# yanzq95/DHD

Measured on AMD Instinct MI355X. Metric: samples/sec (6-cam fwd+bwd) DHD-S view-transform hot path, higher is better.
Workload: dtype f32

## Files before the change

dhd_amd/csrc/sfa_stage.hip:

```cpp
#include <stdlib.h>

#include <type_traits>

#include "sfa_gemm_cu.h"
#include "sfa_gemm_pair.h"
#include "sfa_half.h"
#include "sfa_mfma.h"

using namespace dhd_sfa;

namespace {

constexpr int kEwBlock = 256;
constexpr int kPlaneChunks = 4;
constexpr int kPwBlock = 256;
constexpr int kPwStep = 16;
constexpr int kWgBlock = 512;
constexpr int kWgStride = 33;
constexpr int kWgWorkers = 256;
__host__ __device__ inline long long wg_first_step(long long n, long long w, long long W) { return n * w / W; }
__host__ __device__ inline int wg_owner(long long n, long long s, long long W) { return (int)(((s + 1) * W + n - 1) / n) - 1; }
struct WgFirstStep {
  __host__ __device__ long long operator()(long long n, long long w, long long W) const { return wg_first_step(n, w, W); }
};
inline int wgrad_blocks(int c) { const int ot = c == 128 ? 128 : 256; return (c / ot) * (c / ot); }
inline int wgrad_workers(int c) { const int nob = wgrad_blocks(c); return kWgWorkers / nob > 0 ? kWgWorkers / nob : 1; }
constexpr int kBwdFoldDefault = 7;

__device__ __forceinline__ float block_sum(float v, float* sm) {
  v = group_sum(v, DHD_WAVE);
  const int lane = threadIdx.x & 63, wv = threadIdx.x >> 6;
  __syncthreads();
  if (lane == 0) sm[wv] = v;
  __syncthreads();
  float t = 0.f;
  for (int k = 0; k < (int)(blockDim.x / DHD_WAVE); ++k) t += sm[k];
  return t;
}

template <class TS> constexpr bool kHalfStorage = !std::is_same_v<TS, float>;
template <class TS> constexpr bool kStreamAll = kHalfStorage<TS>;
template <class TS> constexpr int kWideInFlight = kHalfStorage<TS> ? 2 : 1;
template <class TS> constexpr bool kFoldPairwise = !kHalfStorage<TS>;

template <int N> __device__ __forceinline__ void chunk_range(int hw, int* lo, int* hi) {
  static_assert(N == 4 || N == 8, "16 bytes of float32 or of a half type");
  const int n = hw >> (N == 8 ? 3 : 2), per = (n + kPlaneChunks - 1) / kPlaneChunks;
  *lo = blockIdx.x * per;
  *hi = min(n, *lo + per);
}

template <class TO, int N> struct IoVec {
  static constexpr bool k16 = N == kVec16<TO>;
  static_assert(k16 || (N == 4 && sizeof(TO) == 2), "16 bytes, or four elements of a half type");
  using raw = std::conditional_t<k16, raw16<TO>, u32x2>;
  static __device__ __forceinline__ raw ld(const TO* base, size_t i) { return __builtin_nontemporal_load(reinterpret_cast<const raw*>(base) + i); }
  static __device__ __forceinline__ void widen(raw w, float* v) {
    if constexpr (k16) {
      widen16<TO>(w, v);
    } else {
      const f32x2 a = Pair<TO>::widen(w.x), b = Pair<TO>::widen(w.y);
      v[0] = a.x; v[1] = a.y; v[2] = b.x; v[3] = b.y;
    }
  }
  static __device__ __forceinline__ void store(TO* base, size_t i, const float* v) {
    if constexpr (k16) {
      Vec16<TO, true>::store(base, i, v);
    } else {
      typedef TO t4 __attribute__((ext_vector_type(4)));
      const t4 h = {(TO)v[0], (TO)v[1], (TO)v[2], (TO)v[3]};
      __builtin_nontemporal_store(h, reinterpret_cast<t4*>(base) + i);
    }
  }
};

template <int N> __device__ __forceinline__ float tree_sum(const float* v) {
  if constexpr (N == 4) return (v[0] + v[1]) + (v[2] + v[3]);
  else return tree_sum<N / 2>(v) + tree_sum<N / 2>(v + N / 2);
}

template <class TS> __device__ __forceinline__ float fold_sum(float acc, const float* a) {
  if constexpr (kFoldPairwise<TS>) return acc + tree_sum<kVec16<TS>>(a);
#pragma unroll
  for (int j = 0; j < kVec16<TS>; ++j) acc += a[j];
  return acc;
}
template <class TS, class D> __device__ __forceinline__ float fold_dot(float acc, const float* a, D d) {
  if constexpr (kFoldPairwise<TS>) {
    static_assert(kVec16<TS> == 4, "the pairwise fold is written for four elements");
    return acc + ((a[0] * d(0) + a[1] * d(1)) + (a[2] * d(2) + a[3] * d(3)));
  }
#pragma unroll
  for (int j = 0; j < kVec16<TS>; ++j) acc = fmaf(a[j], d(j), acc);
  return acc;
}

template <int K, class Load, class Body> __device__ __forceinline__ void for_each_vector(int lo, int hi, Load load, Body body) {
  int i = lo + threadIdx.x;
  if constexpr (K == 2) {
    for (; i + kEwBlock < hi; i += 2 * kEwBlock) {
      const auto u = load(i), w = load(i + kEwBlock);
      body(u, i);
      body(w, i + kEwBlock);
    }
    if (i < hi) body(load(i), i);
  } else {
    for (; i < hi; i += kEwBlock) body(load(i), i);
  }
}


template <class TS>
__device__ __forceinline__ void plane_mean_block(const TS* __restrict__ x, float* __restrict__ part, int hw, float* sm) {
  constexpr int N = kVec16<TS>;
  using X = Vec16<TS, true>;
  const size_t plane = blockIdx.y;
  const TS* p = x + plane * hw;
  int lo, hi;
  chunk_range<N>(hw, &lo, &hi);
  float a0 = 0.f, a1 = 0.f;
  int i = lo + threadIdx.x;
  for (; i + kEwBlock < hi; i += 2 * kEwBlock) {
    float v[N], w[N];
    X::load(p, i, v);
    X::load(p, (size_t)i + kEwBlock, w);
    a0 += tree_sum<N>(v);
    a1 += tree_sum<N>(w);
  }
  if (i < hi) {
    float v[N];
    X::load(p, i, v);
    a0 += tree_sum<N>(v);
  }
  const float tot = block_sum(a0 + a1, sm);
  if (threadIdx.x == 0) part[plane * kPlaneChunks + blockIdx.x] = tot;
}

__global__ __launch_bounds__(kEwBlock) void plane_mean_kernel(const float* __restrict__ x, float* __restrict__ part, int hw) {
  __shared__ float sm[kEwBlock / DHD_WAVE];
  plane_mean_block(x, part, hw, sm);
}

constexpr int kFcBlock = 1024;
__global__ __launch_bounds__(kFcBlock) void fc_forward_kernel(const float* __restrict__ part, const float* __restrict__ w1,
                                                              const float* __restrict__ b1, const float* __restrict__ w2,
                                                              const float* __restrict__ b2, float* __restrict__ s,
                                                              float* __restrict__ hbuf, float* __restrict__ a,
                                                              float* __restrict__ tab, int c, int r, int hw,
                                                              int* __restrict__ ticks, int n_ticks) {
  extern __shared__ float sh[];
  if (blockIdx.x == 0)
    for (int i = threadIdx.x; i < n_ticks; i += kFcBlock) ticks[i] = 0;
  float* ss = sh;
  float* hh = sh + 2 * c;
  const int b = blockIdx.x, c2 = 2 * c;
  for (int i = threadIdx.x; i < c2; i += kFcBlock) {
    const float* q = part + ((size_t)b * c2 + i) * kPlaneChunks;
    float v = ((q[0] + q[1]) + (q[2] + q[3])) / (float)hw;
    ss[i] = v;
    s[(size_t)b * c2 + i] = v;
  }
  __syncthreads();
  const int lane = threadIdx.x & 63, wv = threadIdx.x >> 6;
  for (int j0 = wv * 4; j0 < r; j0 += 4 * (kFcBlock / DHD_WAVE)) {
    float acc[4] = {0.f, 0.f, 0.f, 0.f};
    for (int i = lane; i < c2; i += DHD_WAVE) {
      const float sv = ss[i];
#pragma unroll
      for (int q = 0; q < 4; ++q)
        if (j0 + q < r) acc[q] = fmaf(w1[(size_t)(j0 + q) * c2 + i], sv, acc[q]);
    }
#pragma unroll
    for (int q = 0; q < 4; ++q) {
      const float t = group_sum(acc[q], DHD_WAVE);
      if (lane == 0 && j0 + q < r) {
        const float v = fmaxf(t + b1[j0 + q], 0.f);
        hh[j0 + q] = v;
        hbuf[(size_t)b * r + j0 + q] = v;
      }
    }
// ... 1337 lines not shown
      constexpr int OT = decltype(ot_c)::value;
      if constexpr (!std::is_same<TS, float>::value) {
        const size_t shmem = (size_t)2 * 4 * 2 * (OT / 32) * 64 * 16;
        return launch_lds<pw_wgrad_h_kernel<TS, OT, V::two, V::relu>>(grid, block, shmem, shmem, st, a0, a1, acoef, a_bs, b0, b1, bcoef,
                                                                     b_bs, partial, c, hw, b, workers);
      } else if (p.wgrad == Wgrad::w3) {
        const size_t shmem = (size_t)2 * 2 * 2 * (OT / 32) * 2 * 64 * 16;
        if (fold.mode != 0) {
          if (nob != 1 || fold.mode != (V::two ? 2 : 1)) return (int)DHD_EUNSUPPORTED;
          return launch_lds<pw_wgrad3_kernel<OT, false, V::two, V::relu, V::two ? 2 : 1>>(grid, block, shmem, shmem, st, a0, a1, acoef, a_bs, b0, b1,
                                                                                         bcoef, b_bs, partial, c, hw, b, workers, fold.aux,
                                                                                         fold.mean, fold.rows);
        }
        return launch_lds<pw_wgrad3_kernel<OT, true, V::two, V::relu>>(grid, block, shmem, shmem, st, a0, a1, acoef, a_bs, b0, b1, bcoef,
                                                                      b_bs, partial, c, hw, b, workers, static_cast<const float*>(nullptr),
                                                                      static_cast<const float*>(nullptr), static_cast<float*>(nullptr));
      } else if (p.wgrad == Wgrad::w6) {
        const size_t shmem = (size_t)2 * 2 * (OT / 32) * 3 * 64 * 16;
        return launch_lds<pw_wgrad6_kernel<OT, true, V::two, V::relu>>(grid, block, shmem, shmem, st, a0, a1, acoef, a_bs, b0, b1, bcoef,
                                                                      b_bs, partial, c, hw, b, workers);
      } else {
        const size_t shmem = (size_t)4 * OT * kWgStride * sizeof(float);
        return launch_lds<pw_wgrad_kernel<OT, true, V::two, V::relu>>(grid, block, shmem, shmem, st, a0, a1, acoef, a_bs, b0, b1, bcoef,
                                                                     b_bs, partial, c, hw, b, workers);
      }
    };
    return ot == 128 ? run(IntC<128>{}) : run(IntC<256>{});
  });
  if (rc != DHD_OK) return rc;
  const int n = c * c;
  hipLaunchKernelGGL(wgrad_reduce_kernel, dim3(dhd_cdiv(n, DHD_WAVE)), dim3(kEwBlock), 0, st, partial, gw, n, workers);
  DHD_LAUNCH_CHECK();
  return DHD_OK;
}

template <class TS>
int launch_mean_pack(const Plan& p, const TS* x, const float* w1, const float* w2, void* const dst[4], float* mean_part, int b,
                     int c, int hw, hipStream_t st) {
  const int blocks_each = dhd_cdiv((c / 32) * (c / 16) * 64, kEwBlock);
  if (p.pack == Pack::cu || p.pack == Pack::res || p.pack == Pack::cuh) {
    PackJob job;
    job.w[0] = w1; job.w[1] = w2;
    for (int i = 0; i < 4; ++i) job.dst[i] = static_cast<u32x4*>(dst[i]);
    job.c = c; job.nt = p.nt; job.cob = p.cob; job.cu = p.pack == Pack::cu ? 1 : 0;
    job.blocks_each = blocks_each;
    const dim3 grid(kPlaneChunks, b * 2 * c + dhd_cdiv(4 * blocks_each, kPlaneChunks));
    hipLaunchKernelGGL(plane_mean_pack_kernel<TS>, grid, dim3(kEwBlock), 0, st, x, mean_part, hw, b * 2 * c, job);
    DHD_LAUNCH_CHECK();
    return DHD_OK;
  }
  if constexpr (std::is_same_v<TS, float>) {
    hipLaunchKernelGGL(plane_mean_kernel, dim3(kPlaneChunks, b * 2 * c), dim3(kEwBlock), 0, st, x, mean_part, hw);
    DHD_LAUNCH_CHECK();
    for (int i = 0; i < 4; ++i) {
      const float* wi = i & 1 ? w2 : w1;
      if (p.pack == Pack::six)
        hipLaunchKernelGGL(pack_weight6_kernel, dim3(blocks_each), dim3(kEwBlock), 0, st, wi, i >> 1, static_cast<u32x4*>(dst[i]), c, p.cot);
      else
        hipLaunchKernelGGL(pack_weight_kernel, dim3(dhd_cdiv(c * c, kEwBlock)), dim3(kEwBlock), 0, st, wi, i >> 1, static_cast<float*>(dst[i]),
                           c, p.cot);
      DHD_LAUNCH_CHECK();
    }
    return DHD_OK;
  }
  return DHD_EINVAL;
}

template <class TS, class TO>
int stage_forward(const Plan& p, const TS* x, const dhd_sfa_weights* w, TO* out, void* saved, void* scratch, int b, int c, int hw,
                  int lo, int hi, double* sync, hipStream_t st) {
  const int r = w->hidden;
  const SavedLayout S = saved_layout(b, c, hw, r, p.storage);
  const ScratchLayout T = scratch_layout(b, c, hw, r, p.storage);
  char* sv = static_cast<char*>(saved);
  char* sc = static_cast<char*>(scratch);
  auto SF = [&](size_t off) { return reinterpret_cast<float*>(sv + off); };
  auto TF = [&](size_t off) { return reinterpret_cast<float*>(sc + off); };
  TS* y1 = reinterpret_cast<TS*>(sv + S.y1);
  TS* y2 = reinterpret_cast<TS*>(sv + S.y2);
  float* stat_part = p.fused_stats ? TF(T.stat_part) : nullptr;
  const dim3 planes(kPlaneChunks, b * c), per_ch(dhd_cdiv(c, kEwBlock));
  const size_t cs = (size_t)c * hw;
  int stat_rows = 0, rc;
  struct Bn {
    const float *shift, *gamma, *beta;
    float *run_mean, *run_var;
    float momentum, eps;
    long long* batches;
    float *mean, *rstd, *scsh;
    double* loc;
  };
  const Bn bn1 = {w->conv1_b, w->bn1_w, w->bn1_b, w->bn1_mean, w->bn1_var, w->momentum1, w->eps1,
                  reinterpret_cast<long long*>(w->bn1_batches), SF(S.mean1), SF(S.rstd1), SF(S.scsh1), reinterpret_cast<double*>(sv + S.loc1)};
  const Bn bn2 = {w->conv2_b, w->bn2_w, w->bn2_b, w->bn2_mean, w->bn2_var, w->momentum2, w->eps2,
                  reinterpret_cast<long long*>(w->bn2_batches), SF(S.mean2), SF(S.rstd2), SF(S.scsh2), reinterpret_cast<double*>(sv + S.loc2)};
  auto publish = [&](const Bn& n, float* tab) {
    hipLaunchKernelGGL(bn_stats_finalize_kernel, dim3(c / 4), dim3(kEwBlock), 0, st, TF(T.stat_part), stat_rows, n.shift, n.gamma, n.beta,
                       n.run_mean, n.run_var, n.momentum, n.eps, n.mean, n.rstd, n.scsh, tab, b, c, hw, sync, n.loc, nullptr, nullptr);
  };
  auto coef = [&](const Bn& n, const TS* y, float* tab) {
    if (!w->training) {
      hipLaunchKernelGGL(bn_eval_coef_kernel, per_ch, dim3(kEwBlock), 0, st, n.gamma, n.beta, n.run_mean, n.run_var, n.eps, n.mean, n.rstd,
                         n.scsh, tab, b, c);
    } else if (p.fused_stats) {
      hipLaunchKernelGGL(bn_stats_finalize_kernel, dim3(c / 4), dim3(kEwBlock), 0, st, TF(T.stat_part), stat_rows, n.shift, n.gamma, n.beta,
                         n.run_mean, n.run_var, n.momentum, n.eps, n.mean, n.rstd, n.scsh, tab, b, c, hw, nullptr, nullptr, sync, n.batches);
    } else if constexpr (std::is_same<TS, float>::value) {
      hipLaunchKernelGGL(moments_kernel, planes, dim3(kEwBlock), 0, st, y, TF(T.part), c, hw);
      hipLaunchKernelGGL(bn_train_finalize_kernel, per_ch, dim3(kEwBlock), 0, st, TF(T.part), b * kPlaneChunks, y, hw, n.gamma, n.beta,
                         n.run_mean, n.run_var, n.momentum, n.eps, n.mean, n.rstd, n.scsh, tab, b, c, hw, n.batches);
    }
  };
  if (sync && !p.fused_stats) return DHD_EUNSUPPORTED;

  if (lo <= 0) {
    void* const dst[4] = {sc + T.wp1, sc + T.wp2, sv + S.wp1t, sv + S.wp2t};
    rc = launch_mean_pack(p, x, w->conv1_w, w->conv2_w, dst, TF(T.mean_part), b, c, hw, st);
    if (rc != DHD_OK) return rc;
    hipLaunchKernelGGL(fc_forward_kernel, dim3(b), dim3(kFcBlock), (size_t)(2 * c + r) * sizeof(float), st, TF(T.mean_part), w->fc1_w,
                       w->fc1_b, w->fc2_w, w->fc2_b, SF(S.s), SF(S.h), SF(S.a1), SF(S.tab_a), c, r, hw, reinterpret_cast<int*>(sv + S.tick),
                       2 * c + kTickWords);
    DHD_LAUNCH_CHECK();
    rc = launch_gemm(p, GemmCall<TS>{kConv1, x, x + cs, 2 * cs, c, SF(S.tab_a), sc + T.wp1, w->conv1_b, nullptr, stat_part, y1},
                     b, c, hw, st, &stat_rows);
    if (rc != DHD_OK) return rc;
    if (sync) {
      publish(bn1, SF(S.tab1));
      DHD_LAUNCH_CHECK();
    }
  }
  if (hi <= 0) return DHD_OK;
  if (lo <= 1) {
    coef(bn1, y1, SF(S.tab1));
    DHD_LAUNCH_CHECK();
    rc = launch_gemm(p, GemmCall<TS>{kConv2, y1, nullptr, cs, c, SF(S.tab1), sc + T.wp2, w->conv2_b,
                                     reinterpret_cast<unsigned*>(sv + S.mask), stat_part, y2},
                     b, c, hw, st, &stat_rows);
    if (rc != DHD_OK) return rc;
    if (sync) {
      publish(bn2, TF(T.tab_g2));
      DHD_LAUNCH_CHECK();
    }
  }
  if (hi <= 1) return DHD_OK;
  coef(bn2, y2, TF(T.tab_g2));
  hipLaunchKernelGGL((blend2_bn_kernel<TS, TO>), planes, dim3(kEwBlock), 0, st, x, SF(S.a1), y2, SF(S.scsh2), out, c, hw);
  DHD_LAUNCH_CHECK();
  return DHD_OK;
}

int bwd_fold_mode() {
  static const int mode = [] {
    const char* e = getenv("DHD_SFA_BWD_FOLD");
    return e != nullptr && e[0] >= '0' && e[0] <= '7' && e[1] == 0 ? e[0] - '0' : kBwdFoldDefault;
  }();
  return mode;
}

int launch_pair(const PairArgs& a, float* gw, int c, hipStream_t st) {
  const size_t shmem = pair_lds_bytes(c);
  int rc;
  if (c == 256) rc = launch_lds<pw_pair_kernel<256, 2, WgFirstStep>>(dim3(kPairGrid), dim3(512), shmem, shmem, st, a);
  else if (c == 128) rc = launch_lds<pw_pair_kernel<128, 2, WgFirstStep>>(dim3(kPairGrid), dim3(256), shmem, shmem, st, a);
  else return DHD_EUNSUPPORTED;
  if (rc != DHD_OK) return rc;
  const int n = c * c;
  hipLaunchKernelGGL(wgrad_reduce_kernel, dim3(dhd_cdiv(n, DHD_WAVE)), dim3(kEwBlock), 0, st, a.partial, gw, n, kPairWorkers);
  DHD_LAUNCH_CHECK();
  return DHD_OK;
}

template <class TS, class TO>
int stage_backward(const Plan& p, const TS* x, const dhd_sfa_weights* w, const void* saved, const TO* gout, TO* gx,
                   const dhd_sfa_grads* grads, void* scratch, int b, int c, int hw, int lo, int hi, double* sync, hipStream_t st) {
  const int r = w->hidden;
  const SavedLayout S = saved_layout(b, c, hw, r, p.storage);
  const ScratchLayout T = scratch_layout(b, c, hw, r, p.storage);
  char* sv = const_cast<char*>(static_cast<const char*>(saved));
  char* sc = static_cast<char*>(scratch);
  auto SF = [&](size_t off) { return reinterpret_cast<float*>(sv + off); };
  auto TF = [&](size_t off) { return reinterpret_cast<float*>(sc + off); };
  const TS* y1 = reinterpret_cast<const TS*>(sv + S.y1);
  const TS* y2 = reinterpret_cast<const TS*>(sv + S.y2);
  TS* g2 = reinterpret_cast<TS*>(sc + T.g2);
  TS* g1 = reinterpret_cast<TS*>(sc + T.g1);
  TS* du = reinterpret_cast<TS*>(sc + T.du);
  unsigned* mask = reinterpret_cast<unsigned*>(sv + S.mask);
  int* tick = reinterpret_cast<int*>(sv + S.tick);
  const dim3 planes(kPlaneChunks, b * c), per_ch(dhd_cdiv(c, kEwBlock));
  const size_t cs = (size_t)c * hw;
  int rc;
  const BnTail tail2 = {sync ? nullptr : tick, w->bn2_w, SF(S.mean2), SF(S.rstd2), TF(T.tab_g2), grads->bn2_w, grads->bn2_b,
                        grads->conv2_b, w->training, b, hw};
  const BnTail tail1 = {sync ? nullptr : tick + c, w->bn1_w, SF(S.mean1), SF(S.rstd1), TF(T.tab_g1), grads->bn1_w, grads->bn1_b,
                        grads->conv1_b, w->training, b, hw};
  auto coef_out = [&](const BnTail& t) {
    hipLaunchKernelGGL(bn_backward_coef_kernel, per_ch, dim3(kEwBlock), 0, st, TF(T.part), t.gamma, t.mean, t.rstd, w->training, t.tab,
                       t.dgamma, t.dbeta, t.dbias, b, c, hw, sync, nullptr, nullptr, nullptr);
  };
  auto coef_in = [&](const BnTail& t, size_t loc, const float* bias) {
    hipLaunchKernelGGL(bn_backward_coef_kernel, per_ch, dim3(kEwBlock), 0, st, TF(T.part), t.gamma, t.mean, t.rstd, w->training, t.tab,
                       t.dgamma, t.dbeta, t.dbias, b, c, hw, nullptr, sync, reinterpret_cast<const double*>(sv + loc), bias);
  };
  if (sync && !p.fused_stats) return DHD_EUNSUPPORTED;
  int fold = 0;
  const int fold_workers = wgrad_workers(c);
  if constexpr (std::is_same_v<TS, float>) {
    const size_t plane = (size_t)b * cs * sizeof(float);
    if (p.gemm == Gemm::cu && p.wgrad == Wgrad::w3 && sync == nullptr && wgrad_blocks(c) == 1 && (size_t)fold_workers * 2 * c * sizeof(float) <= plane &&
        (size_t)(fold_workers + b) * c * sizeof(float) <= plane)
      fold = bwd_fold_mode();
  }
  float* rows1 = reinterpret_cast<float*>(du);
  float* rows2 = reinterpret_cast<float*>(g2);

  if (lo <= 0) {
    hipLaunchKernelGGL((blend2_bn_bwd_kernel<TS, TO>), planes, dim3(kEwBlock), 0, st, x, SF(S.a1), y2, SF(S.scsh2), SF(S.mean2), gout, g2, TF(T.part),
                       TF(T.da1), c, hw, tail2);
    if (sync) coef_out(tail2);
    DHD_LAUNCH_CHECK();
  }
  if (hi <= 0) return DHD_OK;
  if (lo <= 1) {
    if (sync) coef_in(tail2, S.loc2, w->conv2_b);
    DHD_LAUNCH_CHECK();
  }
  if (lo <= 1 && (fold & 4)) {
    if constexpr (std::is_same_v<TS, float>) {
      rc = launch_pair(PairArgs{g2, y2, TF(T.tab_g2), reinterpret_cast<const u32x4*>(sv + S.wp2t), y1, SF(S.scsh1), SF(S.mean1), g1, TF(T.wpart),
                                rows1, hw, b},
                       grads->conv2_w, c, st);
      if (rc != DHD_OK) return rc;
      const BnRowsJob j1 = {tail1.gamma, tail1.mean, tail1.rstd, tail1.tab, tail1.dgamma, tail1.dbeta, tail1.dbias, w->training, b, hw};
      hipLaunchKernelGGL(bn_backward_rows_kernel, dim3(c / 4), dim3(kEwBlock), 0, st, rows1, kPairWorkers, j1, c);
      DHD_LAUNCH_CHECK();
    }
  } else if (lo <= 1 && (fold & 1)) {
    if constexpr (std::is_same_v<TS, float>) {
      rc = launch_gemm(p, GemmCall<TS>{kDgrad2, g2, y2, cs, c, TF(T.tab_g2), sv + S.wp2t, nullptr, mask, nullptr, g1, y1, SF(S.scsh1), CuBlend{}, 0, g2},
                       b, c, hw, st);
      if (rc != DHD_OK) return rc;
      rc = launch_wgrad<TS>(p, kConv2, g2, nullptr, nullptr, cs, y1, nullptr, SF(S.tab1), cs, TF(T.wpart), grads->conv2_w, b, c, hw, st,
                            WgradFold{1, g1, SF(S.mean1), rows1});
      if (rc != DHD_OK) return rc;
      const BnRowsJob j1 = {tail1.gamma, tail1.mean, tail1.rstd, tail1.tab, tail1.dgamma, tail1.dbeta, tail1.dbias, w->training, b, hw};
      hipLaunchKernelGGL(bn_backward_rows_kernel, dim3(c / 4), dim3(kEwBlock), 0, st, rows1, fold_workers, j1, c);
      DHD_LAUNCH_CHECK();
    }
  } else if (lo <= 1) {
    rc = launch_wgrad<TS>(p, kConv2, g2, y2, TF(T.tab_g2), cs, y1, nullptr, SF(S.tab1), cs, TF(T.wpart), grads->conv2_w, b, c, hw, st);
    if (rc != DHD_OK) return rc;
    rc = launch_gemm(p, GemmCall<TS>{kDgrad2, g2, y2, cs, c, TF(T.tab_g2), sv + S.wp2t, nullptr, mask, nullptr, g1, y1, SF(S.scsh1)},
                     b, c, hw, st);
    if (rc != DHD_OK) return rc;
    hipLaunchKernelGGL(pair_sums_kernel<TS>, planes, dim3(kEwBlock), 0, st, g1, y1, SF(S.mean1), TF(T.part), c, hw, tail1);
    if (sync) coef_out(tail1);
    DHD_LAUNCH_CHECK();
  }
  if (hi <= 1) return DHD_OK;
  if (sync) coef_in(tail1, S.loc1, w->conv1_b);
  DHD_LAUNCH_CHECK();
  if (fold & 2) {
    if constexpr (std::is_same_v<TS, float>) {
      rc = launch_gemm(p, GemmCall<TS>{kDgrad1, g1, y1, cs, c, TF(T.tab_g1), sv + S.wp1t, nullptr, nullptr, nullptr, du, nullptr, nullptr, CuBlend{}, 0, g1},
                       b, c, hw, st);
      if (rc != DHD_OK) return rc;
      rc = launch_wgrad<TS>(p, kConv1, g1, nullptr, nullptr, cs, x, x + cs, SF(S.tab_a), 2 * cs, TF(T.wpart), grads->conv1_w, b, c, hw, st,
                            WgradFold{2, du, nullptr, rows2});
      if (rc != DHD_OK) return rc;
      hipLaunchKernelGGL(fc_backward_kernel, dim3(b), dim3(kEwBlock), (size_t)(c + r + kEwBlock) * sizeof(float), st, TF(T.da1), rows2,
                         SF(S.a1), SF(S.h), w->fc1_w, w->fc2_w, TF(T.dpre2), TF(T.dh), TF(T.ds), c, r, fold_workers, (hw + 31) / 32);
    }
  } else {
    rc = launch_wgrad<TS>(p, kConv1, g1, y1, TF(T.tab_g1), cs, x, x + cs, SF(S.tab_a), 2 * cs, TF(T.wpart), grads->conv1_w, b, c, hw, st);
    if (rc != DHD_OK) return rc;
    rc = launch_gemm(p, GemmCall<TS>{kDgrad1, g1, y1, cs, c, TF(T.tab_g1), sv + S.wp1t, nullptr, nullptr, nullptr, du}, b, c, hw, st);
    if (rc != DHD_OK) return rc;
    hipLaunchKernelGGL(blend1_da_kernel<TS>, planes, dim3(kEwBlock), 0, st, x, du, TF(T.da2), c, hw);
    hipLaunchKernelGGL(fc_backward_kernel, dim3(b), dim3(kEwBlock), (size_t)(c + r + kEwBlock) * sizeof(float), st, TF(T.da1), TF(T.da2),
                       SF(S.a1), SF(S.h), w->fc1_w, w->fc2_w, TF(T.dpre2), TF(T.dh), TF(T.ds), c, r, 0, 0);
  }
  const int n_fc = r * 2 * c + c * r + r + c;
  const FcGradJob fcj = {TF(T.dpre2), TF(T.dh), SF(S.h), SF(S.s), grads->fc1_w, grads->fc1_b, grads->fc2_w, grads->fc2_b, b, r};
  const int fc_rows = dhd_cdiv(dhd_cdiv(n_fc, kEwBlock), kPlaneChunks);
  const dim3 planes_fc(kPlaneChunks, b * c + fc_rows);
  hipLaunchKernelGGL((stage_gx_kernel<TS, TO>), planes_fc, dim3(kEwBlock), 0, st, SF(S.a1), y2, SF(S.scsh2), gout, du, TF(T.ds), gx, c, hw, fc_rows, fcj);
  DHD_LAUNCH_CHECK();
  return DHD_OK;
}

inline bool infer_form_exists(const Plan& p, int form) {
  switch (form) {
    case DHD_SFA_INFER_AUTO: case DHD_SFA_INFER_UNFUSED: return true;
    case DHD_SFA_INFER_TWO_PASS: return p.gemm == Gemm::cu || p.gemm == Gemm::cuh;
    case DHD_SFA_INFER_ONE_PASS: return p.gemm == Gemm::cuh;
    default: return false;
  }
}
inline int infer_resolve(const Plan& p, int form) {
  if (form != DHD_SFA_INFER_AUTO) return form;
  if (infer_form_exists(p, DHD_SFA_INFER_ONE_PASS)) return DHD_SFA_INFER_ONE_PASS;
  return infer_form_exists(p, DHD_SFA_INFER_TWO_PASS) ? DHD_SFA_INFER_TWO_PASS : DHD_SFA_INFER_UNFUSED;
}

struct InferLayout {
  size_t wp1, wp2, mean_part, s, h, a1, tab_a, mean1, rstd1, scsh1, tab1, mean2, rstd2, scsh2, tab2, y1, total;
};
inline InferLayout infer_layout(int b, int c, int hw, int r, int storage, bool with_y1) {
  const bool half = storage != DHD_F32;
  const size_t cc = (size_t)c * c;
  InferLayout L;
  size_t o = 0;
  auto take = [&](size_t bytes) { size_t at = o; o += (bytes + 255) & ~(size_t)255; return at; };
  auto f = [&](size_t n) { return take(n * sizeof(float)); };
  L.wp1 = take(half ? 2 * cc : 8 * cc); L.wp2 = take(half ? 2 * cc : 8 * cc);
  L.mean_part = f((size_t)b * 2 * c * kPlaneChunks);
  L.s = f((size_t)b * 2 * c); L.h = f((size_t)b * r); L.a1 = f((size_t)b * c); L.tab_a = f((size_t)b * 3 * c);
  L.mean1 = f(c); L.rstd1 = f(c); L.scsh1 = f(2 * c); L.tab1 = f((size_t)b * 3 * c);
  L.mean2 = f(c); L.rstd2 = f(c); L.scsh2 = f(2 * c); L.tab2 = f((size_t)b * 3 * c);
  L.y1 = take(with_y1 ? (size_t)b * c * hw * (half ? 2 : 4) : 0);
  L.total = o;
  return L;
}

inline size_t infer_scratch_total(const Plan& p, int form, int b, int c, int hw, int r) {
  const int f = infer_resolve(p, form);
  if (f != DHD_SFA_INFER_UNFUSED) return infer_layout(b, c, hw, r, p.storage, f == DHD_SFA_INFER_TWO_PASS).total;
  return saved_layout(b, c, hw, r, p.storage).total + scratch_layout(b, c, hw, r, p.storage).total;
}

template <class TS>
int launch_onepass(const TS* x, const OnePassArgs& A, TS* out, int b, int c, int hw, hipStream_t st) {
  const int max_b = onepass_max_batch(c);
  if (max_b < 1) return DHD_EUNSUPPORTED;
  const int nwt = (hw + kCuhTile - 1) / kCuhTile;
  int cus = cu_count();
  if (cus <= 0) cus = 256;
  for (int b0 = 0; b0 < b; b0 += max_b) {
    const int nb = b - b0 < max_b ? b - b0 : max_b;
    const long total = (long)nb * nwt;
    const int grid = (int)(total < cus ? total : cus);
    OnePassArgs a = A;
    a.tab_a += (size_t)b0 * 3 * c;
    a.a1 += (size_t)b0 * c;
    const TS* xi = x + (size_t)b0 * 2 * c * hw;
    TS* oi = out + (size_t)b0 * c * hw;
    const size_t shmem = onepass_lds_bytes(c, nb);
    const int rc = c == 256 ? launch_lds<sfa_onepass_h_kernel<TS, 16>>(dim3(grid), dim3(kOnePassWaves * 64), shmem, kLdsBytes, st, xi, a, oi, hw, nb)
                            : launch_lds<sfa_onepass_h_kernel<TS, 8>>(dim3(grid), dim3(kOnePassWaves * 64), shmem, kLdsBytes, st, xi, a, oi, hw, nb);
    if (rc != DHD_OK) return rc;
  }
  return DHD_OK;
}

template <class TS, class TO>
int stage_infer(const Plan& p, const TS* x, const dhd_sfa_weights* w, TO* out, void* scratch, int b, int c, int hw, int form,
                hipStream_t st) {
  const int r = w->hidden;
  char* sc = static_cast<char*>(scratch);
  form = infer_resolve(p, form);
  if (form == DHD_SFA_INFER_UNFUSED)
    return stage_forward<TS, TO>(p, x, w, out, sc, sc + saved_layout(b, c, hw, r, p.storage).total, b, c, hw, 0, 2, nullptr, st);
  const InferLayout L = infer_layout(b, c, hw, r, p.storage, form == DHD_SFA_INFER_TWO_PASS);
  auto F = [&](size_t off) { return reinterpret_cast<float*>(sc + off); };
  TS* y1 = reinterpret_cast<TS*>(sc + L.y1);
  const size_t cs = (size_t)c * hw;
  void* const dst[4] = {sc + L.wp1, sc + L.wp2, nullptr, nullptr};
  int rc = launch_mean_pack(p, x, w->conv1_w, w->conv2_w, dst, F(L.mean_part), b, c, hw, st);
  if (rc != DHD_OK) return rc;
  hipLaunchKernelGGL(fc_forward_kernel, dim3(b), dim3(kFcBlock), (size_t)(2 * c + r) * sizeof(float), st, F(L.mean_part), w->fc1_w, w->fc1_b,
                     w->fc2_w, w->fc2_b, F(L.s), F(L.h), F(L.a1), F(L.tab_a), c, r, hw, static_cast<int*>(nullptr), 0);
  DHD_LAUNCH_CHECK();
  const BnEvalJob j1 = {w->bn1_w, w->bn1_b, w->bn1_mean, w->bn1_var, w->eps1, F(L.mean1), F(L.rstd1), F(L.scsh1), F(L.tab1)};
  const BnEvalJob j2 = {w->bn2_w, w->bn2_b, w->bn2_mean, w->bn2_var, w->eps2, F(L.mean2), F(L.rstd2), F(L.scsh2), F(L.tab2)};
  hipLaunchKernelGGL(bn_eval_coef2_kernel, dim3(dhd_cdiv(c, kEwBlock), 2), dim3(kEwBlock), 0, st, j1, j2, b, c);
  DHD_LAUNCH_CHECK();
  if (form == DHD_SFA_INFER_ONE_PASS) {
    if constexpr (std::is_same<TS, float>::value) {
      return DHD_EUNSUPPORTED;
    } else {
      const OnePassArgs A = {F(L.tab_a), F(L.tab1), w->conv1_b, w->conv2_b, F(L.a1), F(L.scsh2), reinterpret_cast<const u32x4*>(sc + L.wp1),
                             reinterpret_cast<const u32x4*>(sc + L.wp2)};
      return launch_onepass<TS>(x, A, reinterpret_cast<TS*>(out), b, c, hw, st);
    }
  }
  rc = launch_gemm(p, GemmCall<TS>{kConv1, x, x + cs, 2 * cs, c, F(L.tab_a), sc + L.wp1, w->conv1_b, nullptr, nullptr, y1}, b, c, hw, st);
  if (rc != DHD_OK) return rc;
  return launch_gemm(p, GemmCall<TS>{kConv2Blend, y1, nullptr, cs, c, F(L.tab1), sc + L.wp2, w->conv2_b, nullptr, nullptr, nullptr, nullptr,
                                     nullptr, CuBlend{x, F(L.a1), F(L.scsh2), out}, w->io_dtype},
                     b, c, hw, st);
}

template <class F>
int with_types(const Plan& p, int io_dtype, F&& f) {
  if (p.storage == DHD_F16) return f((_Float16*)nullptr, (_Float16*)nullptr);
  if (p.storage == DHD_BF16) return f((__bf16*)nullptr, (__bf16*)nullptr);
  if (io_dtype == DHD_F16) return f((float*)nullptr, (_Float16*)nullptr);
  if (io_dtype == DHD_BF16) return f((float*)nullptr, (__bf16*)nullptr);
  return f((float*)nullptr, (float*)nullptr);
}

static int stage_forward_entry(const void* x, const dhd_sfa_weights* w, void* out, void* saved, void* scratch, int b, int c, int hw,
                               int lo, int hi, double* sync, void* stream) {
  if (!x || !w || !saved || !scratch || b <= 0 || (hi == 2 && !out)) return DHD_EINVAL;
  if (!dhd_aligned(16, x, out, saved, scratch)) return DHD_EINVAL;
  if (!stage_supported(c, hw) || w->hidden <= 0) return DHD_EUNSUPPORTED;
  if (!w->fc1_w || !w->fc1_b || !w->fc2_w || !w->fc2_b || !w->conv1_w || !w->conv1_b || !w->bn1_w || !w->bn1_b || !w->conv2_w ||
      !w->conv2_b || !w->bn2_w || !w->bn2_b)
    return DHD_EINVAL;
  if (!w->training && (!w->bn1_mean || !w->bn1_var || !w->bn2_mean || !w->bn2_var)) return DHD_EINVAL;
  Plan p;
  if (int rc = make_plan(w, c, hw, &p); rc != DHD_OK) return rc;
  return with_types(p, w->io_dtype, [&](auto* ts, auto* to) {
    using TS = std::remove_pointer_t<decltype(ts)>;
    using TO = std::remove_pointer_t<decltype(to)>;
// ... 128 lines not shown
```

Measured before the change: 2858.

## Fuse conv1 dgrad and weight-gradient into a single paired MFMA kernel

Adds a pw_pair1 kernel that, per 32-pixel step, rebuilds the BN-backward gradient from g1/y1, computes the conv1 data gradient with split-bf16 MFMA, and accumulates the conv1 weight gradient from the blended input in the same pass, also producing per-row reduction sums for the FC backward. It becomes the new default via fold mode 15. The goal is to avoid separate dgrad and wgrad launches that each reread g1/y1/x from memory. The cost is a much more complex kernel with one block per CU and heavy register and LDS pressure, and the extra fold bit only applies to float storage.

```diff
diff --git a/dhd_amd/csrc/sfa_gemm_pair1.h b/dhd_amd/csrc/sfa_gemm_pair1.h
--- /dev/null
+++ b/dhd_amd/csrc/sfa_gemm_pair1.h
@@ -0,0 +1,273 @@
+#pragma once
+#include "sfa_gemm_pair.h"
+
+namespace dhd_sfa {
+
+inline size_t pair1_lds_bytes(int c) { return pair_lds_bytes(c) + (size_t)c * sizeof(float); }
+
+struct Pair1Args {
+  const float* g;
+  const float* y;
+  const float* coef;
+  const u32x4* wp;
+  const float* x;
+  const float* tab_a;
+  float* out;
+  float* partial;
+  float* rows;
+  int hw, nb;
+};
+
+template <int C, int AUX, class FirstStep, int SAUX = 0, int XAUX = AUX>
+__global__ __launch_bounds__(2 * C, 1) void pw_pair1_kernel(Pair1Args a) {
+  static_assert(C == 128 || C == 256, "C/32 waves, C/64 weight-gradient tiles per wave");
+  constexpr int KS = C / 32, KCN = C / 16, HALF = C / 2;
+  constexpr int TCO = C / 32, TCI = C / 64;
+  constexpr int TA = C / 128, TB = 2, WCI = TCI / TB;
+  constexpr int DIMG = 128 * C, AIMG = 128 * C, BIMG = 64 * C;
+  extern __shared__ __attribute__((aligned(16))) unsigned char pair_lds[];
+  unsigned char* const dimg = pair_lds;
+  unsigned char* const aimg = pair_lds + DIMG;
+  unsigned char* const bimg = pair_lds + DIMG + AIMG;
+  const int tid = threadIdx.x, lane = tid & 63;
+  const int wv = __builtin_amdgcn_readfirstlane(tid >> 6);
+  const int g = lane >> 3, q = lane & 7;
+  float* const patch = reinterpret_cast<float*>(pair_lds + DIMG + AIMG + BIMG) + wv * (16 * kPairPatchPitch);
+  const PairSlot slot = pair_slot((int)blockIdx.x);
+  const int cib = slot.half * HALF;
+  const int hw = a.hw, sps = (hw + 31) >> 5;
+  const long long n_steps = (long long)a.nb * sps;
+  const int first = (int)FirstStep{}(n_steps, slot.worker, kPairWorkers);
+  const int count = (int)FirstStep{}(n_steps, slot.worker + 1, kPairWorkers) - first;
+  const int row_bytes = hw * 4;
+  const unsigned in_bytes = (unsigned)((size_t)C * hw * sizeof(float));
+  const unsigned x_bytes = (unsigned)((size_t)2 * C * hw * sizeof(float));
+
+  u32x4 wh[KS], wm[KS];
+  {
+    const int row = cib + 16 * wv + (lane & 15), kq = lane >> 4;
+#pragma unroll
+    for (int ks = 0; ks < KS; ++ks) {
+      const u32x4* src = a.wp + ((size_t)((row >> 5) * KCN + 2 * ks + (kq >> 1)) * 2) * 64 + (row & 31) + 32 * (kq & 1);
+      wh[ks] = src[0];
+      wm[ks] = src[64];
+    }
+  }
+  const int co0 = 32 * wv + 4 * g;
+  float* const cf_lds = reinterpret_cast<float*>(pair_lds + DIMG + AIMG + BIMG) + (C / 32) * (16 * kPairPatchPitch);
+  float* const ab_lds = cf_lds + 3 * C;
+  for (int i = tid; i < 3 * C; i += 2 * C) cf_lds[i] = a.coef[i];
+  auto load_ab = [&](int b) {
+    if (tid < HALF) {
+      const float* t = a.tab_a + (size_t)b * 3 * C + cib + tid;
+      *reinterpret_cast<f32x2*>(ab_lds + 2 * tid) = f32x2{t[0], t[C]};
+    }
+  };
+  load_ab(min(first / sps, a.nb - 1));
+  const int lda_voff = (co0 * hw + 4 * q) * 4;
+  const int ldb_voff = ((cib + 16 * wv + g) * hw + 4 * q) * 4;
+  const int aw0 = pair_a_write(C, co0, q, 0), bw0 = pair_b_write(C, 16 * wv + g, q, 0);
+  auto xor_c = [](int v, auto cc) {
+    int r;
+    asm("v_xor_b32 %0, %1, %2" : "=v"(r) : "n"(decltype(cc)::value), "v"(v));
+    return r;
+  };
+  const int dw = pair_d_write(co0, 4 * q, 0);
+  const int a_rd = (lane ^ (lane >> 5)) << 4, b_rd = (lane ^ ((lane >> 5) << 1)) << 4;
+
+  f32x16 acc[TA][TB];
+#pragma unroll
+  for (int i = 0; i < TA; ++i)
+#pragma unroll
+    for (int j = 0; j < TB; ++j)
+#pragma unroll
+      for (int e = 0; e < 16; ++e) acc[i][j][e] = 0.f;
+  float fs[2] = {0.f, 0.f};
+  auto flush = [&](int bs) {
+#pragma unroll
+    for (int k = 0; k < 2; ++k) {
+      float v = fs[k];
+      v += __shfl_xor(v, 1, DHD_WAVE);
+      v += __shfl_xor(v, 2, DHD_WAVE);
+      v += __shfl_xor(v, 4, DHD_WAVE);
+      if (q == 0) a.rows[(size_t)(slot.worker + bs) * C + cib + 16 * wv + g + 8 * k] = v;
+      fs[k] = 0.f;
+    }
+  };
+
+  f32x4 rg[4], ry[4], rxb[2], rxv[2];
+  auto issue = [&](int s) {
+    const int b = s / sps, p0 = (s - b * sps) * 32;
+    const __amdgpu_buffer_rsrc_t sg = __builtin_amdgcn_make_buffer_rsrc(const_cast<float*>(a.g + (size_t)b * C * hw), 0, in_bytes, 0x00020000);
+    const __amdgpu_buffer_rsrc_t sy = __builtin_amdgcn_make_buffer_rsrc(const_cast<float*>(a.y + (size_t)b * C * hw), 0, in_bytes, 0x00020000);
+    const __amdgpu_buffer_rsrc_t sx = __builtin_amdgcn_make_buffer_rsrc(const_cast<float*>(a.x + (size_t)b * 2 * C * hw), 0, x_bytes, 0x00020000);
+    const bool okq = p0 + 4 * q < hw;
+    const int va = okq ? lda_voff : lda_voff - 16 * q, vb = okq ? ldb_voff : ldb_voff - 16 * q;
+#pragma unroll
+    for (int j = 0; j < 4; ++j) {
+      rg[j] = __builtin_bit_cast(f32x4, __builtin_amdgcn_raw_buffer_load_b128(sg, va, j * row_bytes + p0 * 4, AUX));
+      ry[j] = __builtin_bit_cast(f32x4, __builtin_amdgcn_raw_buffer_load_b128(sy, va, j * row_bytes + p0 * 4, AUX));
+    }
+#pragma unroll
+    for (int k = 0; k < 2; ++k) {
+      rxb[k] = __builtin_bit_cast(f32x4, __builtin_amdgcn_raw_buffer_load_b128(sx, vb, 8 * k * row_bytes + p0 * 4, XAUX));
+      rxv[k] = __builtin_bit_cast(f32x4, __builtin_amdgcn_raw_buffer_load_b128(sx, vb, (C + 8 * k) * row_bytes + p0 * 4, XAUX));
+    }
+  };
+
+  __builtin_amdgcn_s_waitcnt(0x0F70);
+  cu_lds_barrier();
+  if (count > 0) {
+    issue(first);
+    {
+      const __amdgpu_buffer_rsrc_t ro = __builtin_amdgcn_make_buffer_rsrc(a.out, 0, 16, 0x00020000);
+      store_b128_guarded<0>(u32x4{0u, 0u, 0u, 0u}, ro, 0x7ffffff0, 0);
+      store_b128_guarded<0>(u32x4{0u, 0u, 0u, 0u}, ro, 0x7ffffff0, 0);
+    }
+  }
+  for (int it = 0; it < count; ++it) {
+    const int s = first + it;
+    const int b = s / sps, p0 = (s - b * sps) * 32;
+    const int s_next = first + min(it + 1, count - 1);
+    const bool okq = p0 + 4 * q < hw;
+    float v[4][4];
+    {
+      const f32x4 c0 = *reinterpret_cast<const f32x4*>(cf_lds + co0);
+      const f32x4 c1 = *reinterpret_cast<const f32x4*>(cf_lds + C + co0);
+      const f32x4 c2 = *reinterpret_cast<const f32x4*>(cf_lds + 2 * C + co0);
+#pragma unroll
+      for (int e = 0; e < 4; ++e)
+#pragma unroll
+        for (int j = 0; j < 4; ++j) {
+          float tv = fmaf(c0[j], rg[j][e], c2[j]);
+          tv = fmaf(c1[j], ry[j][e], tv);
+          v[e][j] = okq ? tv : 0.f;
+        }
+    }
+    f32x4 xd[2];
+    float u[2][4];
+#pragma unroll
+    for (int k = 0; k < 2; ++k) {
+      const f32x2 ab = *reinterpret_cast<const f32x2*>(ab_lds + 2 * (16 * wv + g + 8 * k));
+#pragma unroll
+      for (int e = 0; e < 4; ++e) {
+        float tu = fmaf(ab.x, rxb[k][e], 0.f);
+        tu = fmaf(ab.y, rxv[k][e], tu);
+        u[k][e] = okq ? tu : 0.f;
+        xd[k][e] = rxb[k][e] - rxv[k][e];
+      }
+    }
+    __builtin_amdgcn_sched_barrier(0);
+    issue(s_next);
+    __builtin_amdgcn_sched_barrier(0);
+    unsigned h01[4], m01[4], h23[4], m23[4];
+#pragma unroll
+    for (int e = 0; e < 4; ++e) {
+      split2_hm(v[e][0], v[e][1], h01[e], m01[e]);
+      split2_hm(v[e][2], v[e][3], h23[e], m23[e]);
+      const int off = dw + (((e >> 1) * 64 + 8 * (e & 1)) << 4);
+      *reinterpret_cast<u32x2*>(dimg + off) = u32x2{h01[e], h23[e]};
+      *reinterpret_cast<u32x2*>(dimg + off + 2048) = u32x2{m01[e], m23[e]};
+    }
+    {
+      constexpr unsigned LO = 0x05040100u, HI = 0x07060302u;
+      static_for<4>([&](auto jc) {
+        constexpr int j = decltype(jc)::value;
+        const unsigned* hs = j < 2 ? h01 : h23;
+        const unsigned* ms = j < 2 ? m01 : m23;
+        const unsigned sel = (j & 1) ? HI : LO;
+        const u32x2 hq = {__builtin_amdgcn_perm(hs[1], hs[0], sel), __builtin_amdgcn_perm(hs[3], hs[2], sel)};
+        const u32x2 mq = {__builtin_amdgcn_perm(ms[1], ms[0], sel), __builtin_amdgcn_perm(ms[3], ms[2], sel)};
+        const int aw = xor_c(aw0, std::integral_constant<int, (j << 4)>{});
+        *reinterpret_cast<u32x2*>(aimg + aw) = hq;
+        *reinterpret_cast<u32x2*>(aimg + aw + 1024) = mq;
+      });
+    }
+    static_for<2>([&](auto kc) {
+      constexpr int k = decltype(kc)::value;
+      unsigned uh01, um01, uh23, um23;
+      split2_hm(u[k][0], u[k][1], uh01, um01);
+      split2_hm(u[k][2], u[k][3], uh23, um23);
+      const int bw = xor_c(bw0, std::integral_constant<int, (k << 7)>{});
+      *reinterpret_cast<u32x2*>(bimg + bw) = u32x2{uh01, uh23};
+      *reinterpret_cast<u32x2*>(bimg + bw + 1024) = u32x2{um01, um23};
+    });
+    cu_lds_barrier();
+
+    f32x4 dacc[2] = {{0.f, 0.f, 0.f, 0.f}, {0.f, 0.f, 0.f, 0.f}};
+#pragma unroll
+    for (int ks = 0; ks < KS; ++ks)
+#pragma unroll
+      for (int nt = 0; nt < 2; ++nt) {
+        const u32x4 bh = *reinterpret_cast<const u32x4*>(dimg + pair_d_read(ks, 0, nt, lane));
+        const u32x4 bm = *reinterpret_cast<const u32x4*>(dimg + pair_d_read(ks, 1, nt, lane));
+        dacc[nt] = mfma16_bf16(wm[ks], bh, dacc[nt]);
+        dacc[nt] = mfma16_bf16(wh[ks], bm, dacc[nt]);
+        dacc[nt] = mfma16_bf16(wh[ks], bh, dacc[nt]);
+      }
+    {
+      const int wco = wv / WCI, wci = wv % WCI;
+#pragma unroll
+      for (int k2 = 0; k2 < 2; ++k2) {
+        u32x4 fb[TB][2];
+#pragma unroll
+        for (int j = 0; j < TB; ++j)
+#pragma unroll
+          for (int t = 0; t < 2; ++t) fb[j][t] = *reinterpret_cast<const u32x4*>(bimg + ((((k2 * TCI + TB * wci + j) * 2 + t) * 64) << 4) + (b_rd ^ (k2 << 6)));
+#pragma unroll
+        for (int i = 0; i < TA; ++i) {
+          u32x4 fa[2];
+#pragma unroll
+          for (int t = 0; t < 2; ++t) fa[t] = *reinterpret_cast<const u32x4*>(aimg + ((((k2 * TCO + TA * wco + i) * 2 + t) * 64) << 4) + (a_rd ^ (k2 << 5)));
+#pragma unroll
+          for (int j = 0; j < TB; ++j) acc[i][j] = mfma_bf16(fa[1], fb[j][0], acc[i][j]);
+#pragma unroll
+          for (int j = 0; j < TB; ++j) acc[i][j] = mfma_bf16(fa[0], fb[j][1], acc[i][j]);
+#pragma unroll
+          for (int j = 0; j < TB; ++j) acc[i][j] = mfma_bf16(fa[0], fb[j][0], acc[i][j]);
+        }
+      }
+    }
+    {
+      const int col = lane & 15, prow = 4 * (lane >> 4);
+#pragma unroll
+      for (int nt = 0; nt < 2; ++nt)
+#pragma unroll
+        for (int i = 0; i < 4; ++i) patch[(prow + i) * kPairPatchPitch + 4 * (col & 7) + 2 * nt + (col >> 3)] = dacc[nt][i];
+      const __amdgpu_buffer_rsrc_t ro = __builtin_amdgcn_make_buffer_rsrc(a.out + (size_t)b * C * hw, 0, in_bytes, 0x00020000);
+      const int voff = okq ? ldb_voff : 0x7ffffff0;
+#pragma unroll
+      for (int k = 0; k < 2; ++k) {
+        const f32x4 o = *reinterpret_cast<const f32x4*>(patch + (g + 8 * k) * kPairPatchPitch + 4 * q);
+        const f32x4 d = xd[k];
+        const float t1 = (o.x * d.x + o.y * d.y) + (o.z * d.z + o.w * d.w);
+        fs[k] += okq ? t1 : 0.f;
+        store_b128_guarded<SAUX>(__builtin_bit_cast(u32x4, o), ro, voff, 8 * k * row_bytes + p0 * 4);
+      }
+    }
+    const int b_next = s_next / sps;
+    if (b_next != b) {
+      flush(b);
+      load_ab(b_next);
+    }
+    cu_lds_barrier();
+  }
+
+  {
+    const int wco = wv / WCI, wci = wv % WCI;
+    float* po = a.partial + (size_t)slot.worker * C * C;
+#pragma unroll
+    for (int i = 0; i < TA; ++i)
+#pragma unroll
+      for (int j = 0; j < TB; ++j)
+#pragma unroll
+        for (int e = 0; e < 16; ++e) {
+          const int co = 32 * (TA * wco + i) + (e & 3) + 8 * (e >> 2) + 4 * (lane >> 5);
+          const int ci = cib + 32 * (TB * wci + j) + (lane & 31);
+          po[(size_t)co * C + ci] = acc[i][j][e];
+        }
+  }
+  flush(count > 0 ? (first + count - 1) / sps : min(first / sps, a.nb - 1));
+}
+
+}
diff --git a/dhd_amd/csrc/sfa_stage.hip b/dhd_amd/csrc/sfa_stage.hip
--- a/dhd_amd/csrc/sfa_stage.hip
+++ b/dhd_amd/csrc/sfa_stage.hip
@@ -4,6 +4,7 @@
 
 #include "sfa_gemm_cu.h"
 #include "sfa_gemm_pair.h"
+#include "sfa_gemm_pair1.h"
 #include "sfa_half.h"
 #include "sfa_mfma.h"
 
@@ -25,7 +26,7 @@
 };
 inline int wgrad_blocks(int c) { const int ot = c == 128 ? 128 : 256; return (c / ot) * (c / ot); }
 inline int wgrad_workers(int c) { const int nob = wgrad_blocks(c); return kWgWorkers / nob > 0 ? kWgWorkers / nob : 1; }
-constexpr int kBwdFoldDefault = 7;
+constexpr int kBwdFoldDefault = 15;
 
 __device__ __forceinline__ float block_sum(float v, float* sm) {
   v = group_sum(v, DHD_WAVE);
@@ -1669,7 +1670,10 @@
 int bwd_fold_mode() {
   static const int mode = [] {
     const char* e = getenv("DHD_SFA_BWD_FOLD");
-    return e != nullptr && e[0] >= '0' && e[0] <= '7' && e[1] == 0 ? e[0] - '0' : kBwdFoldDefault;
+    if (e == nullptr || e[0] < '0' || e[0] > '9') return kBwdFoldDefault;
+    if (e[1] == 0) return e[0] - '0';
+    if (e[0] == '1' && e[1] >= '0' && e[1] <= '5' && e[2] == 0) return 10 + (e[1] - '0');
+    return kBwdFoldDefault;
   }();
   return mode;
 }
@@ -1679,6 +1683,19 @@
   int rc;
   if (c == 256) rc = launch_lds<pw_pair_kernel<256, 2, WgFirstStep>>(dim3(kPairGrid), dim3(512), shmem, shmem, st, a);
   else if (c == 128) rc = launch_lds<pw_pair_kernel<128, 2, WgFirstStep>>(dim3(kPairGrid), dim3(256), shmem, shmem, st, a);
+  else return DHD_EUNSUPPORTED;
+  if (rc != DHD_OK) return rc;
+  const int n = c * c;
+  hipLaunchKernelGGL(wgrad_reduce_kernel, dim3(dhd_cdiv(n, DHD_WAVE)), dim3(kEwBlock), 0, st, a.partial, gw, n, kPairWorkers);
+  DHD_LAUNCH_CHECK();
+  return DHD_OK;
+}
+
+int launch_pair1(const Pair1Args& a, float* gw, int c, hipStream_t st) {
+  const size_t shmem = pair1_lds_bytes(c);
+  int rc;
+  if (c == 256) rc = launch_lds<pw_pair1_kernel<256, 2, WgFirstStep>>(dim3(kPairGrid), dim3(512), shmem, shmem, st, a);
+  else if (c == 128) rc = launch_lds<pw_pair1_kernel<128, 2, WgFirstStep>>(dim3(kPairGrid), dim3(256), shmem, shmem, st, a);
   else return DHD_EUNSUPPORTED;
   if (rc != DHD_OK) return rc;
   const int n = c * c;
@@ -1777,7 +1794,15 @@
   if (hi <= 1) return DHD_OK;
   if (sync) coef_in(tail1, S.loc1, w->conv1_b);
   DHD_LAUNCH_CHECK();
-  if (fold & 2) {
+  if (fold & 8) {
+    if constexpr (std::is_same_v<TS, float>) {
+      rc = launch_pair1(Pair1Args{g1, y1, TF(T.tab_g1), reinterpret_cast<const u32x4*>(sv + S.wp1t), x, SF(S.tab_a), du, TF(T.wpart), rows2, hw, b},
+                        grads->conv1_w, c, st);
+      if (rc != DHD_OK) return rc;
+      hipLaunchKernelGGL(fc_backward_kernel, dim3(b), dim3(kEwBlock), (size_t)(c + r + kEwBlock) * sizeof(float), st, TF(T.da1), rows2,
+                         SF(S.a1), SF(S.h), w->fc1_w, w->fc2_w, TF(T.dpre2), TF(T.dh), TF(T.ds), c, r, kPairWorkers, (hw + 31) / 32);
+    }
+  } else if (fold & 2) {
     if constexpr (std::is_same_v<TS, float>) {
       rc = launch_gemm(p, GemmCall<TS>{kDgrad1, g1, y1, cs, c, TF(T.tab_g1), sv + S.wp1t, nullptr, nullptr, nullptr, du, nullptr, nullptr, CuBlend{}, 0, g1},
                        b, c, hw, st);
```

Result: faster. 2952 (median of 6 runs) (+3.3%).
